# mynameisfiber/baton

Measured on NVIDIA H100. Metric: federated local samples/sec (whole box), ResNet-18 FedAvg, synthetic non-IID 32x32 shards, higher is better.
Workload: dtype bf16

## Files before the change

### baton_b200/csrc/bindings.cpp

```cpp
#include <ATen/cuda/CUDAContext.h>
#include <c10/cuda/CUDAGuard.h>
#include <torch/extension.h>

#include <optional>
#include <vector>

#include "launch.h"

namespace {

inline cudaStream_t cur_stream() { return at::cuda::getCurrentCUDAStream().stream(); }
inline void check(int rc, const char* what) {
  TORCH_CHECK(rc == 0, "baton_b200::", what, " failed with code ", rc,
              rc > 0 ? std::string(" (") + cudaGetErrorString(static_cast<cudaError_t>(rc)) + ")" : std::string());
}
inline const void* cptr(const at::Tensor& t) { return t.data_ptr(); }
inline void* ptr(at::Tensor& t) { return t.data_ptr(); }
template <class T>
inline T* opt_ptr(const std::optional<at::Tensor>& t) {
  return (t.has_value() && t->defined()) ? reinterpret_cast<T*>(t->data_ptr()) : nullptr;
}
#define CHECK_CUDA(x) TORCH_CHECK((x).is_cuda(), #x " must be a CUDA tensor")

inline const float* prox_anchor(const std::optional<at::Tensor>& anchor, int64_t numel, const at::Tensor& hyper) {
// ... 230 lines not shown
  TORCH_CHECK(rows > 0 && out.numel() % rows == 0, "conv_halo: out must hold [N*Ho*Wo, Nout] elements");
  const int64_t nout = out.numel() / rows;
  TORCH_CHECK(w.numel() == (dgrad ? c * 9 * nout : nout * 9 * c), "conv_halo: w must be [Cout, 9*Cin]");
  TORCH_CHECK(dgrad ? !col_stats.has_value()
                    : (!col_stats.has_value() || (col_stats->scalar_type() == at::kFloat && col_stats->numel() >= 2 * nout)),
              "conv_halo: col_stats is a [2 Cout] fp32 buffer of the forward");
  const c10::cuda::CUDAGuard guard(src.device());
  const int rc = b200_conv_halo(cptr(src), cptr(w), ptr(out), static_cast<int>(src.size(0)), static_cast<int>(src.size(1)),
                                static_cast<int>(src.size(2)), static_cast<int>(c), static_cast<int>(nout),
                                static_cast<int>(stride), dgrad ? 1 : 0, static_cast<int>(mc), opt_ptr<float>(col_stats),
                                cur_stream());
  if (rc == -2) return false;
  check(rc, "conv_halo");
  return true;
}
bool conv_igemm_dgrad_s2(const at::Tensor& dy, const at::Tensor& w, at::Tensor dx, int64_t kh, int64_t kw,
                         const std::vector<int64_t>& ntaps, const std::vector<int64_t>& taps, int64_t force_bn) {
  CHECK_CUDA(dy); CHECK_CUDA(w); CHECK_CUDA(dx);
  TORCH_CHECK(dy.scalar_type() == at::kBFloat16 && w.scalar_type() == at::kBFloat16 && dx.scalar_type() == at::kBFloat16 &&
              dy.dim() == 4 && dx.dim() == 4 && dy.is_contiguous() && w.is_contiguous() && dx.is_contiguous());
  TORCH_CHECK(ntaps.size() == 4 && taps.size() == 16, "conv_igemm_dgrad_s2: 4 classes x 4 taps");
  int nt[4], tw[16];
  for (int i = 0; i < 4; ++i) nt[i] = static_cast<int>(ntaps[i]);
  for (int i = 0; i < 16; ++i) tw[i] = static_cast<int>(taps[i]);
  const c10::cuda::CUDAGuard guard(dy.device());
  const int rc = b200_conv_igemm_dgrad_s2(cptr(dy), cptr(w), ptr(dx), static_cast<int>(dx.size(0)),
                                          static_cast<int>(dx.size(1)), static_cast<int>(dx.size(2)),
                                          static_cast<int>(dx.size(3)), static_cast<int>(dy.size(3)), static_cast<int>(kh),
                                          static_cast<int>(kw), static_cast<int>(dy.size(1)), static_cast<int>(dy.size(2)),
                                          nt, tw, static_cast<int>(force_bn), cur_stream());
  if (rc == -2) return false;
  check(rc, "conv_igemm_dgrad_s2");
  return true;
}
bool conv_igemm_wgrad(const at::Tensor& dy, const at::Tensor& x, at::Tensor dw, int64_t cout, int64_t kh, int64_t kw,
                      int64_t stride, int64_t pad, int64_t ho, int64_t wo, int64_t split_k, int64_t force_bn,
                      const std::optional<at::Tensor>& sgd_theta, const std::optional<at::Tensor>& sgd_theta_bf16,
                      const std::optional<at::Tensor>& sgd_mom, const std::optional<at::Tensor>& sgd_hyper,
                      bool sgd_nesterov, const std::optional<at::Tensor>& sgd_anchor,
                      const std::optional<at::Tensor>& sgd_corr, const std::optional<at::Tensor>& sgd_v) {
  CHECK_CUDA(dy); CHECK_CUDA(x); CHECK_CUDA(dw);
  TORCH_CHECK(x.scalar_type() == at::kBFloat16 && dy.scalar_type() == at::kBFloat16 && dw.scalar_type() == at::kFloat &&
              x.dim() == 4 && x.is_contiguous() && dy.is_contiguous());
  const c10::cuda::CUDAGuard guard(x.device());
  const std::optional<B200SgdEpilogue> sgd =
      sgd_epilogue(sgd_theta, sgd_theta_bf16, sgd_mom, sgd_hyper, sgd_nesterov, sgd_anchor, sgd_corr, sgd_v);
  const int rc = b200_conv_igemm_wgrad(cptr(dy), cptr(x), dw.data_ptr<float>(), static_cast<int>(x.size(0)),
                                       static_cast<int>(x.size(1)), static_cast<int>(x.size(2)), static_cast<int>(x.size(3)),
                                       static_cast<int>(cout), static_cast<int>(kh), static_cast<int>(kw),
                                       static_cast<int>(stride), static_cast<int>(pad), static_cast<int>(ho),
                                       static_cast<int>(wo), static_cast<int>(split_k), static_cast<int>(force_bn),
                                       sgd ? &*sgd : nullptr, cur_stream());
  if (rc == -2 || rc == B200_SGD_EPILOGUE_DECLINED) return false;
  check(rc, "conv_igemm_wgrad");
  return true;
}

void gemm_fp8(const at::Tensor& a, const at::Tensor& b, at::Tensor d, const std::optional<at::Tensor>& bias,
              const std::optional<at::Tensor>& sfa, const std::optional<at::Tensor>& sfb, int64_t M, int64_t N, int64_t K,
              int64_t lda, int64_t ldb, int64_t ldd, int64_t act, int64_t split_k, bool accumulate, double alpha) {
  CHECK_CUDA(a); CHECK_CUDA(b); CHECK_CUDA(d);
  TORCH_CHECK(a.element_size() == 1 && b.element_size() == 1, "gemm_fp8 operands must be 1-byte (e4m3)");
  const c10::cuda::CUDAGuard guard(a.device());
  check(b200_gemm_fp8(cptr(a), cptr(b), ptr(d), opt_ptr<const float>(bias), opt_ptr<const void>(sfa),
                      opt_ptr<const void>(sfb), M, N, K, lda, ldb, ldd, d.scalar_type() == at::kFloat, act, split_k,
                      accumulate, static_cast<float>(alpha), cur_stream()),
// ... 865 lines not shown
                                       loss_acc.data_ptr<float>(), opt_ptr<float>(logits_out), static_cast<int>(x.size(0)),
                                       static_cast<int>(x.size(1)), static_cast<int>(w.size(0)), cur_stream());
  if (rc == -2) return false;
  check(rc, "linear_xent_eval");
  return true;
}
void mse(const at::Tensor& pred, const at::Tensor& target, const std::optional<at::Tensor>& dpred, at::Tensor loss_acc,
         double grad_scale) {
  CHECK_CUDA(pred);
  TORCH_CHECK(target.scalar_type() == at::kFloat && target.numel() == pred.numel());
  const c10::cuda::CUDAGuard guard(pred.device());
  const int in32 = pred.scalar_type() == at::kFloat;
  const int out32 = dpred.has_value() && dpred->defined() && dpred->scalar_type() == at::kFloat;
  check(b200_mse(pred.data_ptr(), in32, target.data_ptr<float>(), opt_ptr<void>(dpred), out32,
                 loss_acc.data_ptr<float>(), pred.numel(), static_cast<float>(grad_scale), cur_stream()),
        "mse");
}

}

PYBIND11_MODULE(TORCH_EXTENSION_NAME, m) {
  m.doc() = "baton_b200 sm_90a kernels";
  m.attr("MAX_RANKS") = B200_MAX_RANKS;
  m.def("gemm", &gemm);
  m.def("trace_set", &trace_set);
  m.def("attention_fwd", &attention_fwd);
  m.def("attention_bwd", &attention_bwd);
  m.def("bn_bwd_cluster", &bn_bwd_cluster);
  m.def("im2col_tma_probe", &im2col_tma_probe);
  m.def("conv_igemm_fwd", &conv_igemm_fwd);
  m.def("conv_igemm_wgrad", &conv_igemm_wgrad);
  m.def("conv_igemm_dgrad", &conv_igemm_dgrad);
  m.def("conv_igemm_dgrad_s2", &conv_igemm_dgrad_s2);
  m.def("conv_halo", &conv_halo);
  m.def("gemm_batched", &gemm_batched);
  m.def("gemm_fp8", &gemm_fp8);
  m.def("quant_mx_rows", &quant_mx_rows);
  m.def("quant_mx_cols", &quant_mx_cols);
  m.def("fused_sgd", &fused_sgd);
  m.def("fused_sgd_segments", &fused_sgd_segments);
  m.def("weighted_sum", &weighted_sum);
  m.def("fold_client", &fold_client);
  m.def("scaffold_corr", &scaffold_corr);
  m.def("scaffold_dc", &scaffold_dc);
  m.def("cast", &cast);
  m.def("gather_rows", &gather_rows);
  m.def("gather_augment", &gather_augment);
  m.def("gather_mix", &gather_mix);
  m.def("colsum", &colsum);
  m.def("add_bf16", &add_bf16);
  m.def("relu_bwd", &relu_bwd);
  m.def("gelu", &gelu);
  m.def("gelu_bwd", &gelu_bwd);
  m.def("pad_rows", &pad_rows);
  m.def("embedding_bwd", &embedding_bwd);
  m.def("fedavg_allreduce", &fedavg_allreduce);
  m.def("fedavg_allreduce_robust", &fedavg_allreduce_robust);
  m.def("fedavg_allreduce_krum", &fedavg_allreduce_krum);
  m.attr("KRUM_MAX_CTAS") = B200_KRUM_MAX_CTAS;
  m.attr("KRUM_PAIRS") = B200_KRUM_PAIRS;
  m.attr("KRUM_REPORT") = B200_KRUM_REPORT;
  m.def("fedavg_allreduce_topk", &fedavg_allreduce_topk);
  m.def("fedavg_allreduce_local", &fedavg_allreduce_local);
  m.def("topk_pack", &topk_pack);
  m.def("topk_fold", &topk_fold);
  m.def("nonzero_pack", &nonzero_pack);
// ... 31 lines not shown
```

### baton_b200/csrc/gemm_wgmma.cu

```cuda
#define B200_TU_TAG 1
#include "ptx.cuh"
#include "epilogue.cuh"
#include "launch.h"
#include "pdl.cuh"
#include "sgd.cuh"

namespace b200 {

constexpr int BM = 128;
constexpr int BK = 64;
constexpr int WG_K = 16;
constexpr int GEMM_THREADS = 384;
constexpr int CONSUMER_WARPS = 8;
constexpr int CONSUMER_THREADS = 32 * CONSUMER_WARPS;
constexpr int MAX_STAGES = 8;
constexpr int S2_MAX_TAPS = 4;

struct GemmParams {
  int M, N, K;
  void* D;
  long long ldd;
  const float* bias;
  int out_fp32;
  int act;
  float* col_stats;
  int a_mn, b_mn;
  int k_tiles_per_split;
  int atomic_out;
  int cluster_k;
  int stages;
  const uint32_t* tile_flags;
  uint32_t flag_epoch;
  long long flag_elem_off;
  int flag_tile_elems;
  long long flag_bias_off;
  long long ldb;
  float alpha;
  int batched, batch_inner;
  int batch_count;
  long long d_outer, d_inner;
  int conv_ho, conv_wo;
  int conv_stride, conv_pad;
  int conv_kw;
  int conv_cin;
  int conv_taps;
  int conv_ncol;
  const uint32_t* flag_epoch_ptr;
  const float* sgd_hyper = nullptr;
  float* sgd_theta = nullptr;
  __nv_bfloat16* sgd_wb = nullptr;
  float* sgd_mom = nullptr;
  int sgd_nesterov = 0;
  int conv_h = 0, conv_w = 0;
  int s2_ntaps[4] = {0, 0, 0, 0};
  int s2_tap[4][S2_MAX_TAPS] = {};
  const float* bn_scale = nullptr;
  const float* bn_shift = nullptr;
  const __nv_bfloat16* residual = nullptr;
  long long ldr = 0;
  const float* sgd_anchor = nullptr;
  const float* sgd_corr = nullptr;
  float* sgd_v = nullptr;
};

__device__ __forceinline__ void wait_arrival_flags(const uint32_t* flags, long long e0, long long e1, int granule,
                                                   uint32_t need) {
  for (long long t = e0 / granule; t <= e1 / granule; ++t) {
    unsigned long long spins = 0;
    while (static_cast<int32_t>(ld_acquire_sys(flags + t) - need) < 0) {
      if (++spins > (1ull << 26)) break;
    }
  }
}

template <int BN>
struct SmemLayout {
  static constexpr int A_BYTES = BM * BK * 2;
  static constexpr int B_BYTES = BN * BK * 2;
  static constexpr int STAGE_BYTES = A_BYTES + B_BYTES;
  static constexpr int PART_PITCH = BN + 4;
  static constexpr int PART_BYTES = BM * PART_PITCH * 4;
};

__device__ __forceinline__ float apply_act(float v, int act) {
  if (act == 1) return fmaxf(v, 0.f);
  if (act == 2) {
    const float k0 = 0.7978845608028654f, k1 = 0.044715f;
    float t = tanhf(k0 * (v + k1 * v * v * v));
    return 0.5f * v * (1.f + t);
  }
  return v;
}

__device__ __forceinline__ float4 ld_dsmem_f4(uint32_t local_smem_addr, uint32_t cta_rank) {
  uint32_t remote;
// ... 256 lines not shown
__device__ __forceinline__ int s2_ntaps(const GemmParams& p, int cls) {
  int n = 0;
#pragma unroll
  for (int c = 0; c < 4; ++c) n = c == cls ? p.s2_ntaps[c] : n;
  return n;
}
__device__ __forceinline__ int s2_tap(const GemmParams& p, int cls, int slot) {
  int w = 0;
#pragma unroll
  for (int c = 0; c < 4; ++c)
#pragma unroll
    for (int t = 0; t < S2_MAX_TAPS; ++t) w = (c == cls && t == slot) ? p.s2_tap[c][t] : w;
  return w;
}
__device__ __forceinline__ int s2_dx_row(const GemmParams& p, int cls, int m) {
  if (m >= p.M) return -1;
  const int hw = p.conv_ho * p.conv_wo;
  const int n = m / hw, r = m - n * hw;
  const int i = r / p.conv_wo, j = r - i * p.conv_wo;
  const int h = 2 * i + (cls >> 1), w = 2 * j + (cls & 1);
  return (h < p.conv_h && w < p.conv_w) ? (n * p.conv_h + h) * p.conv_w + w : -1;
}
template <int BN>
__device__ __forceinline__ void s2_load_ktile(const CUtensorMap* tmA, const CUtensorMap* tmB, const GemmParams& p,
                                              uint8_t* sa, uint8_t* sb, uint64_t* bar, int cls, int kt, int m0, int n0) {
  const int cblocks = p.conv_cin >> 6;
  const int slot = kt / cblocks, cb = kt - slot * cblocks;
  const int tw = s2_tap(p, cls, slot);
  const int q0 = m0 % p.conv_wo, t0 = m0 / p.conv_wo;
  tma_load_im2col_4d(sa, tmA, bar, cb * 64, q0, t0 % p.conv_ho, t0 / p.conv_ho, (tw >> 24) & 0xff, (tw >> 16) & 0xff);
  const int wcol = (tw & 0xffff) * p.conv_ncol + n0;
#pragma unroll
  for (int j = 0; j < BN / 64; ++j) tma_load_2d(sb + j * 8192, tmB, bar, wcol + j * 64, cb * 64);
}

template <int BN, int STAGES, int CONV = 0, bool SGD = false, bool AFFINE = false, bool PROX = false, bool SCAF = false,
          bool ADAM = false>
__global__ void __launch_bounds__(GEMM_THREADS, 1)
gemm_bf16_fixed_kernel(const __grid_constant__ CUtensorMap tmA, const __grid_constant__ CUtensorMap tmB,
                         const GemmParams p) {
  using L = SmemLayout<BN>;
  static_assert(STAGES * L::STAGE_BYTES >= L::PART_BYTES, "the drained ring must hold the fp32 accumulator tile");
  extern __shared__ __align__(1024) uint8_t smem_raw[];
  uint8_t* smem = reinterpret_cast<uint8_t*>((reinterpret_cast<uintptr_t>(smem_raw) + 1023) & ~uintptr_t(1023));
  uint64_t* full_bar = reinterpret_cast<uint64_t*>(smem + STAGES * L::STAGE_BYTES);
  uint64_t* empty_bar = full_bar + STAGES;
  float* cstat = reinterpret_cast<float*>(empty_bar + STAGES);

  griddep_launch_dependents();
  const int warp = threadIdx.x >> 5;
  int m0 = blockIdx.y * BM;
  const int cls = CONV == 4 ? s2_class(p, m0) : 0;
  const int n0 = blockIdx.x * BN;
  const int k_tiles_total = CONV == 4 ? s2_ntaps(p, cls) * (p.conv_cin >> 6) : (p.K + BK - 1) / BK;
  const int bz_outer = p.batched ? static_cast<int>(blockIdx.z) / p.batch_inner : 0;
  const int bz_inner = p.batched ? static_cast<int>(blockIdx.z) % p.batch_inner : 0;
  const int kt_begin = p.batched ? 0 : blockIdx.z * p.k_tiles_per_split;
  int kt_end = kt_begin + p.k_tiles_per_split;
  if (kt_end > k_tiles_total) kt_end = k_tiles_total;
  const int num_kt = kt_end - kt_begin;

  if (warp == 0 && elect_one()) {
    tma_prefetch_desc(&tmA);
    tma_prefetch_desc(&tmB);
    for (int s = 0; s < STAGES; ++s) {
      mbar_init(&full_bar[s], 1);
// ... 18 lines not shown
        fence_proxy_async_all();
      }
      TRACE_POINT();
      for (int i = 0; i < num_kt; ++i) {
        const int s = i % STAGES;
        const uint32_t ph = (i / STAGES) & 1;
        mbar_wait(&empty_bar[s], ph ^ 1);
        uint8_t* sa = smem + s * L::STAGE_BYTES;
        uint8_t* sb = sa + L::A_BYTES;
        const int k0 = (kt_begin + i) * BK;
        if constexpr (CONV == 2) {
          const int live = (p.N - n0 + 63) / 64 < BN / 64 ? (p.N - n0 + 63) / 64 : BN / 64;
          mbar_expect_tx(&full_bar[s], L::A_BYTES + live * 8192);
        } else {
          mbar_expect_tx(&full_bar[s], L::STAGE_BYTES);
        }
        if (p.batched) {
          if (!p.a_mn) {
            tma_load_4d(sa, &tmA, &full_bar[s], k0, m0, bz_inner, bz_outer);
          } else {
#pragma unroll
            for (int j = 0; j < BM / 64; ++j)
              tma_load_4d(sa + j * 8192, &tmA, &full_bar[s], m0 + j * 64, k0, bz_inner, bz_outer);
          }
          if (!p.b_mn) {
            tma_load_4d(sb, &tmB, &full_bar[s], k0, n0, bz_inner, bz_outer);
          } else {
#pragma unroll
            for (int j = 0; j < BN / 64; ++j)
              tma_load_4d(sb + j * 8192, &tmB, &full_bar[s], n0 + j * 64, k0, bz_inner, bz_outer);
          }
        } else if constexpr (CONV == 4) {
          s2_load_ktile<BN>(&tmA, &tmB, p, sa, sb, &full_bar[s], cls, kt_begin + i, m0, n0);
        } else {
        if constexpr (CONV == 1 || CONV == 3) {
          const int kt = kt_begin + i;
          const int cblocks = p.conv_cin >> 6;
          const int tap = kt / cblocks, cb = kt - tap * cblocks;
          const int fr = tap / p.conv_kw, fs = tap - fr * p.conv_kw;
          const int q0 = m0 % p.conv_wo, t0 = m0 / p.conv_wo;
          tma_load_im2col_4d(sa, &tmA, &full_bar[s], cb * 64, q0 * p.conv_stride - p.conv_pad,
                             (t0 % p.conv_ho) * p.conv_stride - p.conv_pad, t0 / p.conv_ho, fs, fr);
        } else if (!p.a_mn) {
          tma_load_2d(sa, &tmA, &full_bar[s], k0, m0);
        } else {
#pragma unroll
          for (int j = 0; j < BM / 64; ++j)
            tma_load_2d(sa + j * 8192, &tmA, &full_bar[s], m0 + j * 64, k0);
        }
        if constexpr (CONV == 2) {
          const int q0 = k0 % p.conv_wo, t0 = k0 / p.conv_wo;
          const int w0 = q0 * p.conv_stride - p.conv_pad, h0 = (t0 % p.conv_ho) * p.conv_stride - p.conv_pad;
          const int img = t0 / p.conv_ho;
#pragma unroll
          for (int j = 0; j < BN / 64; ++j) {
            const int col = n0 + j * 64;
            if (col < p.N) {
              const int tap = col / p.conv_cin, c = col - tap * p.conv_cin;
              const int fr = tap / p.conv_kw, fs = tap - fr * p.conv_kw;
              tma_load_im2col_4d(sb + j * 8192, &tmB, &full_bar[s], c, w0, h0, img, fs, fr);
            }
          }
        } else if constexpr (CONV == 3) {
          const int kt = kt_begin + i;
          const int cblocks = p.conv_cin >> 6;
          const int tap = kt / cblocks, cb = kt - tap * cblocks;
// ... 78 lines not shown
          _Pragma("unroll") for (int j = 0; j < 32; ++j) if (col0 + j < p.N) atomicAdd(d + j, v[j]);
        }
      } else if (p.out_fp32) {
        float* d = reinterpret_cast<float*>(drow) + col0;
        if (full && vec_ok) {
#pragma unroll
          for (int j = 0; j < 32; j += 4)
            *reinterpret_cast<float4*>(d + j) = make_float4(v[j], v[j + 1], v[j + 2], v[j + 3]);
        } else {
          _Pragma("unroll") for (int j = 0; j < 32; ++j) if (col0 + j < p.N) d[j] = v[j];
        }
      } else {
        __nv_bfloat16* d = reinterpret_cast<__nv_bfloat16*>(drow) + col0;
        if (full && vec_ok) {
#pragma unroll
          for (int j = 0; j < 32; j += 8) {
            uint4 o;
            o.x = pack_bf16x2(v[j], v[j + 1]);
            o.y = pack_bf16x2(v[j + 2], v[j + 3]);
            o.z = pack_bf16x2(v[j + 4], v[j + 5]);
            o.w = pack_bf16x2(v[j + 6], v[j + 7]);
            *reinterpret_cast<uint4*>(d + j) = o;
          }
        } else {
          _Pragma("unroll") for (int j = 0; j < 32; ++j) if (col0 + j < p.N) d[j] = __float2bfloat16_rn(v[j]);
        }
      }
    }
    if (threadIdx.x == 128) TRACE_POINT();
    if (want_stats) {
      named_bar_sync(1, CONSUMER_THREADS);
      for (int i = threadIdx.x - 128; i < 2 * BN; i += CONSUMER_THREADS) {
        const int col = i < BN ? i : i - BN;
        if (n0 + col < p.N)
          atomicAdd(p.col_stats + (i < BN ? 0 : p.N) + n0 + col,
                    cstat[i] + cstat[2 * BN + i] + cstat[4 * BN + i] + cstat[6 * BN + i]);
      }
    }
  }
}


constexpr int EPI_PITCH = 144;
constexpr int EPI_WARP_BYTES = 32 * EPI_PITCH;

template <int BN>
__device__ __forceinline__ void epilogue_tile(const GemmParams& p, const float* acc_tile, int q, int half, int m0,
                                              int n0, uint8_t* stage, bool vec_ok, size_t d_off = 0) {
  using L = SmemLayout<BN>;
  const int lane = static_cast<int>(lane_id());
  const int row = m0 + q * 32 + lane;
  const float* arow = acc_tile + (q * 32 + lane) * L::PART_PITCH;
  const int elt = p.out_fp32 ? 4 : 2;
  const bool fast = vec_ok && !p.atomic_out && (p.N % 8 == 0);
  if (!fast) {
#pragma unroll 1
    for (int c = half * 32; c < BN; c += 64) {
      uint32_t r[32];
      acc_ld_row32(arow + c, r);
      const int col0 = n0 + c;
      if (col0 >= p.N) continue;
      float v[32];
#pragma unroll
      for (int j = 0; j < 32; ++j) v[j] = __uint_as_float(r[j]);
      if (p.col_stats != nullptr) accumulate_col_stats(p, col0, v);
      if (row >= p.M) continue;
      store_row_chunk<32>(p, row, col0, v, vec_ok, d_off);
// ... 180 lines not shown
  }
  __syncthreads();
  griddep_wait();

  if (warp == 0) {
    if (elect_one()) {
      if (p.tile_flags != nullptr) {
        const int rows_here = (p.N - n0) < BN ? (p.N - n0) : BN;
        const uint32_t need = p.flag_epoch_ptr != nullptr ? *reinterpret_cast<const volatile uint32_t*>(p.flag_epoch_ptr)
                                                          : p.flag_epoch;
        wait_arrival_flags(p.tile_flags, p.flag_elem_off + static_cast<long long>(n0) * p.ldb,
                           p.flag_elem_off + static_cast<long long>(n0 + rows_here) * p.ldb - 1, p.flag_tile_elems, need);
        if (p.flag_bias_off >= 0)
          wait_arrival_flags(p.tile_flags, p.flag_bias_off + n0, p.flag_bias_off + n0 + rows_here - 1,
                             p.flag_tile_elems, need);
        fence_proxy_async_all();
      }
      int s = 0;
      uint32_t ph = 0;
      for (int i = 0; i < num_kt; ++i) {
        mbar_wait(&empty_bar[s], ph ^ 1);
        uint8_t* sa = smem + s * L::STAGE_BYTES;
        uint8_t* sb = sa + L::A_BYTES;
        const int k0 = (kt_begin + i) * BK;
        mbar_expect_tx(&full_bar[s], L::STAGE_BYTES);
        if constexpr (CONV == 1 || CONV == 3) {
          const int kt = kt_begin + i;
          const int cblocks = p.conv_cin >> 6;
          const int tap = kt / cblocks, cb = kt - tap * cblocks;
          const int fr = tap / p.conv_kw, fs = tap - fr * p.conv_kw;
          const int q0 = m0 % p.conv_wo, t0 = m0 / p.conv_wo;
          tma_load_im2col_4d(sa, &tmA, &full_bar[s], cb * 64, q0 * p.conv_stride - p.conv_pad,
                             (t0 % p.conv_ho) * p.conv_stride - p.conv_pad, t0 / p.conv_ho, fs, fr);
        } else if (!p.a_mn) {
          tma_load_2d(sa, &tmA, &full_bar[s], k0, m0);
        } else {
#pragma unroll
          for (int j = 0; j < BM / 64; ++j)
            tma_load_2d(sa + j * 8192, &tmA, &full_bar[s], m0 + j * 64, k0);
        }
        if constexpr (CONV == 3) {
          const int kt = kt_begin + i;
          const int cblocks = p.conv_cin >> 6;
          const int tap = kt / cblocks, cb = kt - tap * cblocks;
          const int wcol = (p.conv_taps - 1 - tap) * p.conv_ncol + n0;
#pragma unroll
          for (int j = 0; j < BN / 64; ++j) tma_load_2d(sb + j * 8192, &tmB, &full_bar[s], wcol + j * 64, cb * 64);
        } else if (!p.b_mn) {
          tma_load_2d(sb, &tmB, &full_bar[s], k0, n0);
        } else {
#pragma unroll
          for (int j = 0; j < BN / 64; ++j) tma_load_2d(sb + j * 8192, &tmB, &full_bar[s], n0 + j * 64, k0);
        }
        if (++s == STAGES) { s = 0; ph ^= 1; }
      }
    }
  } else if (warp >= 4) {
    const int ew = warp - 4;
    float acc[BN / 2];
    int s = 0;
    uint32_t ph = 0;
    consume_ktiles<BN>(acc, smem, STAGES, full_bar, empty_bar, s, ph, num_kt, p.a_mn, p.b_mn, ew >> 2);
    named_bar_sync(1, CONSUMER_THREADS);
    float* part = reinterpret_cast<float*>(smem);
    wg_store_acc<BN>(acc, part, L::PART_PITCH, 64 * (ew >> 2));
    if constexpr (!CLUSTER) {
      named_bar_sync(1, CONSUMER_THREADS);
      const int q = ew & 3;
      constexpr int NCHUNK = BN / 32;
      const int c_begin = (ew < 4 ? 0 : (NCHUNK + 1) / 2) * 32, c_end = (ew < 4 ? (NCHUNK + 1) / 2 : NCHUNK) * 32;
      const int lrow = q * 32 + static_cast<int>(lane_id());
      const int row = m0 + lrow;
      const size_t elt = p.out_fp32 ? 4 : 2;
      const bool vec_ok = ((reinterpret_cast<uintptr_t>(p.D) & 15) == 0) && ((p.ldd * elt) % 16 == 0);
#pragma unroll 1
      for (int c = c_begin; c < c_end; c += 32) {
        const int col0 = n0 + c;
        if (row >= p.M || col0 >= p.N) continue;
        uint32_t r[32];
        acc_ld_row32(part + lrow * L::PART_PITCH + c, r);
// ... 28 lines not shown
          v[4] += b.x; v[5] += b.y; v[6] += b.z; v[7] += b.w;
        }
        const int row = m0 + lrow, col0 = n0 + c;
        if (want_stats) {
#pragma unroll
          for (int j = 0; j < 8; ++j) {
            const float rnd = __bfloat162float(__float2bfloat16_rn(v[j]));
            cs[j] += rnd;
            cq[j] = fmaf(rnd, rnd, cq[j]);
          }
        }
        if (row < p.M && col0 < p.N) store_row_chunk<8, AFFINE>(p, row, col0, v, vec_ok);
      }
      if (want_stats) {
#pragma unroll
        for (int j = 0; j < 8; ++j) {
#pragma unroll
          for (int o = CG; o < 32; o <<= 1) {
            cs[j] += __shfl_xor_sync(0xffffffffu, cs[j], o);
            cq[j] += __shfl_xor_sync(0xffffffffu, cq[j], o);
          }
        }
        const int wq = t >> 5, ln = t & 31;
        if (ln < CG) {
#pragma unroll
          for (int j = 0; j < 8; ++j) {
            cstat[wq * 2 * BN + ln * 8 + j] = cs[j];
            cstat[wq * 2 * BN + BN + ln * 8 + j] = cq[j];
          }
        }
        named_bar_sync(2, 128);
        for (int i = t; i < 2 * BN; i += 128) {
          const int col = i < BN ? i : i - BN;
          if (n0 + col < p.N) {
            const float v = cstat[i] + cstat[2 * BN + i] + cstat[4 * BN + i] + cstat[6 * BN + i];
            atomicAdd(p.col_stats + (i < BN ? 0 : p.N) + n0 + col, v);
          }
        }
      }
    }
    cluster_sync_all();
  }
}


typedef CUresult (*EncodeTiledFn)(CUtensorMap*, CUtensorMapDataType, cuuint32_t, void*, const cuuint64_t*,
                                  const cuuint64_t*, const cuuint32_t*, const cuuint32_t*, CUtensorMapInterleave,
                                  CUtensorMapSwizzle, CUtensorMapL2promotion, CUtensorMapFloatOOBfill);

static EncodeTiledFn get_encode_fn() {
  static thread_local bool ctx_bound = false;
  if (!ctx_bound) {
    cudaFree(nullptr);
    ctx_bound = true;
  }
  static EncodeTiledFn fn = nullptr;
  if (fn == nullptr) {
    void* ptr = nullptr;
    cudaDriverEntryPointQueryResult qres;
    cudaError_t e = cudaGetDriverEntryPoint("cuTensorMapEncodeTiled", &ptr, cudaEnableDefault, &qres);
    if (e != cudaSuccess || qres != cudaDriverEntryPointSuccess || ptr == nullptr) return nullptr;
    fn = reinterpret_cast<EncodeTiledFn>(ptr);
  }
  return fn;
}

static int make_map(CUtensorMap* map, const void* base, long long rows, long long cols, long long ld, int box_cols,
// ... 425 lines not shown
  int max_taps = 0;
  for (int c = 0; c < 4; ++c) {
    if (ntaps[c] < 0 || ntaps[c] > S2_MAX_TAPS) return -2;
    for (int t = 0; t < ntaps[c]; ++t) {
      const int tw = taps[c * S2_MAX_TAPS + t];
      if (tw < 0 || (tw & 0xffff) >= KH * KW) return -2;
      p.s2_tap[c][t] = tw;
    }
    p.s2_ntaps[c] = ntaps[c];
    max_taps = ntaps[c] > max_taps ? ntaps[c] : max_taps;
  }
  if (max_taps == 0) return -2;
  const int bn = clamp_bn(force_bn > 0 ? force_bn : (Cin > 64 ? 128 : 64));
  CUtensorMap ta, tb;
  int rc = b200_encode_map_im2col_bf16(&ta, dy, N, Ho, Wo, Cout, 1, 1, 1, 0, 64, BM);
  if (rc) return rc;
  rc = make_map(&tb, w, Cout, static_cast<long long>(KH) * KW * Cin, static_cast<long long>(KH) * KW * Cin, 64, BK);
  if (rc) return rc;
  const int k_tiles = max_taps * (Cout / 64);
  p.M = static_cast<int>(M); p.N = Cin; p.K = k_tiles * BK; p.D = dx; p.ldd = Cin; p.bias = nullptr; p.out_fp32 = 0;
  p.act = 0; p.a_mn = 0; p.b_mn = 1; p.k_tiles_per_split = k_tiles; p.cluster_k = 1; p.atomic_out = 0;
  p.col_stats = nullptr;
  p.tile_flags = nullptr; p.flag_epoch = 0; p.alpha = 1.0f; p.flag_elem_off = 0; p.flag_tile_elems = 0;
  p.ldb = static_cast<long long>(KH) * KW * Cin;
  p.flag_bias_off = -1; p.flag_epoch_ptr = nullptr;
  p.batched = 0; p.batch_inner = 1; p.batch_count = 1; p.d_outer = 0; p.d_inner = 0;
  p.conv_ho = Ho; p.conv_wo = Wo; p.conv_stride = 2; p.conv_pad = 0; p.conv_kw = KW; p.conv_cin = Cout;
  p.conv_taps = KH * KW; p.conv_ncol = Cin; p.conv_h = H; p.conv_w = W;
  dim3 grid((Cin + bn - 1) / bn, static_cast<unsigned>(4 * tiles_m), 1);
  if (bn == 128) return launch_fixed<128, 6, 4>(ta, tb, p, grid, stream);
  return launch_fixed<64, 8, 4>(ta, tb, p, grid, stream);
}

extern "C" int b200_conv_igemm_wgrad(const void* dy, const void* x, float* dw, int N, int H, int W, int Cin, int Cout,
                                     int KH, int KW, int stride, int pad, int Ho, int Wo, int split_k, int force_bn,
                                     const B200SgdEpilogue* sgd, cudaStream_t stream) {
  using namespace b200;
  const long long Mp = static_cast<long long>(N) * Ho * Wo;
  const int Kc = KH * KW * Cin;
  if (Mp <= 0 || Cout <= 0) return 0;
  if (Cin % 64 != 0 || Cout % 8 != 0 || Mp > (1ll << 30) || (reinterpret_cast<uintptr_t>(x) & 15) ||
      (reinterpret_cast<uintptr_t>(dy) & 15) || (reinterpret_cast<uintptr_t>(dw) & 15))
    return -2;
  const int bn = clamp_bn(force_bn > 0 ? force_bn : (Kc > 64 ? 128 : 64));
  CUtensorMap ta, tb;
  int rc = make_map(&ta, dy, Mp, Cout, Cout, 64, BK);
  if (rc) return rc;
  rc = b200_encode_map_im2col_bf16(&tb, x, N, H, W, Cin, KH, KW, stride, pad, 64, 64);
  if (rc) return rc;
  const int k_tiles = static_cast<int>((Mp + BK - 1) / BK);
  if (split_k < 1) split_k = 1;
  if (split_k > k_tiles) split_k = k_tiles;
  const int per = (k_tiles + split_k - 1) / split_k;
  split_k = (k_tiles + per - 1) / per;
  if (sgd != nullptr && split_k != 1) return B200_SGD_EPILOGUE_DECLINED;
  GemmParams p;
  if (sgd != nullptr) set_sgd_epilogue(p, *sgd);
  p.M = Cout; p.N = Kc; p.K = static_cast<int>(Mp); p.D = dw; p.ldd = Kc; p.bias = nullptr; p.out_fp32 = 1; p.act = 0;
  p.a_mn = 1; p.b_mn = 1; p.k_tiles_per_split = per; p.cluster_k = 1; p.atomic_out = 1;
  p.col_stats = nullptr;
  p.tile_flags = nullptr; p.flag_epoch = 0; p.alpha = 1.0f; p.flag_elem_off = 0; p.flag_tile_elems = 0; p.ldb = Kc;
  p.flag_bias_off = -1; p.flag_epoch_ptr = nullptr;
  p.batched = 0; p.batch_inner = 1; p.batch_count = 1; p.d_outer = 0; p.d_inner = 0;
  p.stages = 4;
  p.conv_ho = Ho; p.conv_wo = Wo; p.conv_stride = stride; p.conv_pad = pad; p.conv_kw = KW; p.conv_cin = Cin;
  p.conv_taps = KH * KW; p.conv_ncol = Cin;
// ... 11 lines not shown
```

### baton_b200/csrc/launch.h

```cpp
#pragma once
#include <cuda_runtime.h>
#include <stdint.h>

#define B200_MAX_RANKS 16

extern "C" {

struct B200SgdEpilogue {
  float* theta;
  void* theta_bf16;
  float* mom;
  const float* hyper;
  int nesterov;
  const float* anchor;
  const float* corr;
  float* v;
};
#define B200_SGD_EPILOGUE_DECLINED (-6)

struct B200AffineEpilogue {
  const float* scale;
  const float* shift;
  const void* residual;
  long long ldr;
  int relu;
};
#define B200_AFFINE_EPILOGUE_DECLINED (-7)

int b200_gemm_bf16(const void* a, const void* b, void* d, const float* bias, int M, int N, int K, long long lda,
                   long long ldb, long long ldd, int a_mn, int b_mn, int out_fp32, int act, int split_k, int accumulate,
                   float alpha, const uint32_t* tile_flags, uint32_t flag_epoch, long long flag_elem_off, int flag_tile_elems,
                   long long flag_bias_off, int force_bn, float* col_stats, const uint32_t* flag_epoch_ptr,
                   const B200SgdEpilogue* sgd, const B200AffineEpilogue* affine, cudaStream_t stream);
int b200_gemm_bf16_batched(const void* a, const void* b, void* d, int M, int N, int K, long long lda, long long ldb,
                           long long ldd, int a_mn, int b_mn, int out_fp32, int act, float alpha, int n_outer,
                           int n_inner, long long a_outer, long long a_inner, long long b_outer, long long b_inner,
                           long long d_outer, long long d_inner, int accumulate, cudaStream_t stream);
int b200_attention_fwd(const void* qkv, void* out, void* probs, int B, int S, int H, int dh, float scale,
                       cudaStream_t stream);
int b200_attention_bwd(const void* qkv, const void* dout, const void* probs, void* dqkv, int B, int S, int H, int dh,
                       float scale, cudaStream_t stream);
int b200_conv_igemm_fwd(const void* x, const void* w, void* y, int N, int H, int W, int Cin, int Cout, int KH, int KW,
                        int stride, int pad, int Ho, int Wo, int cluster_k, int force_bn, float* col_stats,
                        const B200AffineEpilogue* affine, cudaStream_t stream);
int b200_conv_igemm_dgrad(const void* dy, const void* w, void* dx, int N, int H, int W, int Cin, int Cout, int KH, int KW,
                          int pad, int Ho, int Wo, int cluster_k, int force_bn, cudaStream_t stream);
int b200_conv_igemm_dgrad_s2(const void* dy, const void* w, void* dx, int N, int H, int W, int Cin, int Cout, int KH,
                             int KW, int Ho, int Wo, const int* ntaps, const int* taps, int force_bn, cudaStream_t stream);
int b200_conv_igemm_wgrad(const void* dy, const void* x, float* dw, int N, int H, int W, int Cin, int Cout, int KH, int KW,
                          int stride, int pad, int Ho, int Wo, int split_k, int force_bn, const B200SgdEpilogue* sgd,
                          cudaStream_t stream);
int b200_conv_halo(const void* src, const void* w, void* out, int N, int H, int W, int C, int Nout, int stride,
                   int dgrad, int mc, float* col_stats, cudaStream_t stream);
int b200_im2col_tma_probe(const void* x, void* col, int N, int H, int W, int C, int KH, int KW, int stride, int pad,
                          int Ho, int Wo, cudaStream_t stream);
int b200_gemm_fp8(const void* a, const void* b, void* d, const float* bias, const void* sfa, const void* sfb, int M, int N,
                  int K, long long lda, long long ldb, long long ldd, int out_fp32, int act, int split_k, int accumulate,
                  float alpha, cudaStream_t stream);
int b200_quant_mx_rows(const void* x, void* q, void* sf, long long R, int C, long long ld_in, int Cp, cudaStream_t stream);
int b200_quant_mx_cols(const void* x, void* q, void* sf, long long R, int C, long long ld_in, long long Rp,
                       cudaStream_t stream);
int b200_gemm_simt(const void* a, const void* b, void* d, const float* bias, int M, int N, int K, long long lda,
                   long long ldb, long long ldd, int a_mn, int b_mn, int out_fp32, int act, int accumulate,
                   float alpha, cudaStream_t stream);

int b200_fused_sgd(float* w, float* g, float* mom, void* w_bf16, long long n, const float* hyper, int zero_grad,
                   int nesterov, const unsigned long long* wire_slot, const float* pack_global,
                   const float* pack_scale, long long n_pack, int wire_fp32, const float* prox_anchor,
                   const float* corr, float* adam_v, cudaStream_t stream);
int b200_fused_sgd_segments(float* w, float* g, float* mom, void* w_bf16, const long long* segments, int n_seg,
                            const float* hyper, int nesterov, const float* prox_anchor, const float* corr,
                            float* adam_v, cudaStream_t stream);
int b200_scaffold_corr(float* corr, const float* c, const float* ci, long long n, cudaStream_t stream);
int b200_scaffold_dc(float* up, float* ci, const float* c, const float* global_w, const float* theta, long long n,
                     float inv_k_eta, int first, cudaStream_t stream);
int b200_fold_client(float* acc, float* theta, const float* global_w, void* w_bf16, float* mom, long long n_mom, long long n,
                     float nk, int mode, int reset, cudaStream_t stream);
int b200_weighted_sum(void* dst, const void* const* srcs, const float* weights, int n_src, long long n, int dtype,
                      cudaStream_t stream);
int b200_cast_f32_bf16(const float* src, void* dst, long long n, cudaStream_t stream);
int b200_cast_bf16_f32(const void* src, float* dst, long long n, cudaStream_t stream);
// ... 182 lines not shown
```

### baton_b200/ops/functional.py

```python
from __future__ import annotations

import collections
import functools
from typing import List, Optional, Sequence, Tuple

import torch

from ._ext import load

BF16 = torch.bfloat16
NUM_SMS = 132


def _pitch(t: torch.Tensor) -> int:
    assert t.dim() == 2 and (t.stride(1) == 1 or t.shape[1] == 1), "GEMM operand must have unit inner stride"
    return t.stride(0) if t.shape[0] > 1 else max(t.stride(0), t.shape[1])


def _tma_ok(t: torch.Tensor) -> bool:
    return t.dtype == BF16 and _pitch(t) % 8 == 0 and t.data_ptr() % 16 == 0


def pick_bn(M: int, N: int) -> int:
    m_tiles = (M + 127) // 128
# ... 377 lines not shown
    gk = {}
    if gate is not None and form != "centre":
        gk = dict(flags=gate["flags"], flag_epoch_word=gate["epoch_word"], flag_elem_off=gate["elem_off"],
                  flag_tile_elems=gate["tile_elems"], force_bn=pick_bn(a.shape[0], w2d.shape[0]))
    return gemm(a, plan.weight(w2d), col_stats=col_stats, affine=affine, **gk), a


HALO_BM = 64
_HALO_MAX_SMEM = 227 * 1024
_HALO_FORMS = ((1, 64), (1, 128), (2, 64))


def halo_smem_bytes(h: int, w: int, c: int = 64, stride: int = 1) -> int:
    ho, wo = conv_out_size(h, 3, stride, 1), conv_out_size(w, 3, stride, 1)
    box = (HALO_BM // (ho * wo)) * (stride * (ho - 1) + 3) * (stride * (wo - 1) + 3) * 128
    k_tiles = 9 * (c // 64)
    return c // 64 * round_up(box, 1024) + k_tiles * 8192 + round_up(1 + k_tiles, 16) * 8 + 4 * 64 * 4 + 1024


def halo_eligible(kh: int, kw: int, stride: int, pad: int, c: int, h: int, w: int,
                  affine: Optional[dict] = None, dgrad: bool = False) -> bool:
    if kh != 3 or kw != 3 or pad != 1 or (stride, c) not in _HALO_FORMS or (dgrad and stride != 1):
        return False
    hw = conv_out_size(h, 3, stride, 1) * conv_out_size(w, 3, stride, 1)
    return (hw <= HALO_BM and HALO_BM % hw == 0 and affine is None and
            halo_smem_bytes(h, w, c, stride) <= _HALO_MAX_SMEM)


def halo_cluster(m_rows: int) -> int:
    tiles = (m_rows + HALO_BM - 1) // HALO_BM
    return 4 if tiles % 4 == 0 else 2 if tiles % 2 == 0 else 1


def _conv_path(path: Optional[str], eligible: bool) -> str:
    if path is None:
        return "halo" if eligible else "im2col"
    if path not in ("halo", "im2col"):
        raise ValueError("path must be None, 'halo' or 'im2col', not {!r}".format(path))
    if path == "halo" and not eligible:
        raise ValueError("the halo kernel does not take this convolution (see halo_eligible)")
    return path


def conv_igemm_fwd(x: torch.Tensor, w2d: torch.Tensor, kh: int, kw: int, stride: int, pad: int,
                   col_stats: Optional[torch.Tensor] = None, affine: Optional[dict] = None,
                   cluster_k: Optional[int] = None, force_bn: int = 0,
                   out: Optional[torch.Tensor] = None, path: Optional[str] = None,
                   mc: Optional[int] = None) -> Optional[torch.Tensor]:
    n, h, w, c = x.shape
    cout = w2d.shape[0]
    if c % 64 or w2d.shape[1] != kh * kw * c or not x.is_contiguous() or not w2d.is_contiguous():
        return None
    ho, wo = conv_out_size(h, kh, stride, pad), conv_out_size(w, kw, stride, pad)
    M, K = n * ho * wo, kh * kw * c
    halo = halo_eligible(kh, kw, stride, pad, c, h, w, affine) and cout % 8 == 0
    if _conv_path(path, halo) == "halo":
        y = out if out is not None else torch.empty((M, cout), dtype=BF16, device=x.device)
        if not load().conv_halo(x, w2d, y, stride, False, mc or halo_cluster(M), col_stats):
            raise RuntimeError("conv_halo declined a convolution halo_eligible admits")
        return y
    bn = force_bn or pick_bn(M, cout)
    if cluster_k is None:
        cluster_k = pick_cluster_k(M, cout, K, bn)
    y = out if out is not None else torch.empty((M, cout), dtype=BF16, device=x.device)
    af = affine or {}
    ok = load().conv_igemm_fwd(x, w2d, y, kh, kw, stride, pad, ho, wo, cluster_k, bn, col_stats, af.get("scale"),
                               af.get("shift"), af.get("residual"), bool(af.get("relu", False)))
    return y if ok else None


S2_MAX_TAPS = 4


def conv_s2_dgrad_taps(kh: int, kw: int, pad: int, ho: int, wo: int) -> Optional[List[List[Tuple[int, int, int]]]]:
    classes = []
    for a in (0, 1):
        for b in (0, 1):
            taps = []
            for r in range(kh):
                if (a + pad - r) % 2:
                    continue
                dp = (a + pad - r) // 2
                for s in range(kw):
                    if (b + pad - s) % 2:
                        continue
                    dq = (b + pad - s) // 2
                    if dp < 0 or dq < 0:
                        return None
                    if dp < ho and dq < wo:
                        taps.append((r * kw + s, dp, dq))
            if len(taps) > S2_MAX_TAPS:
                return None
            classes.append(taps)
    return classes


def conv_igemm_dgrad(dy: torch.Tensor, w2d: torch.Tensor, in_shape, kh: int, kw: int, pad: int, stride: int = 1,
                     out: Optional[torch.Tensor] = None, path: Optional[str] = None,
                     mc: Optional[int] = None, cluster_k: Optional[int] = None) -> Optional[torch.Tensor]:
    n, h, w, c = in_shape
    cout = dy.shape[-1]
    if c % 64 or cout % 64 or w2d.shape[1] != kh * kw * c or not dy.is_contiguous() or not w2d.is_contiguous():
        return None
    if _conv_path(path, halo_eligible(kh, kw, stride, pad, cout, h, w, dgrad=True)) == "halo":
        dx = out if out is not None else torch.empty((n, h, w, c), dtype=BF16, device=dy.device)
        if not load().conv_halo(dy, w2d, dx, 1, True, mc or halo_cluster(n * h * w), None):
            raise RuntimeError("conv_halo declined a convolution halo_eligible admits")
        return dx
    if stride == 1:
        M, K = n * h * w, kh * kw * cout
        bn = pick_bn(M, c)
        dx = out if out is not None else torch.empty((n, h, w, c), dtype=BF16, device=dy.device)
        if cluster_k is None:
            cluster_k = pick_cluster_k(M, c, K, bn)
        ok = load().conv_igemm_dgrad(dy, w2d, dx, kh, kw, pad, cluster_k, bn)
        return dx if ok else None
    if stride != 2:
        return None
    ho, wo = dy.shape[1], dy.shape[2]
    classes = conv_s2_dgrad_taps(kh, kw, pad, ho, wo)
    if classes is None:
        return None
    bn = pick_bn(4 * n * ho * wo, c)
    words = [[t | dp << 16 | dq << 24 for t, dp, dq in taps] + [0] * (S2_MAX_TAPS - len(taps)) for taps in classes]
    dx = out if out is not None else torch.empty((n, h, w, c), dtype=BF16, device=dy.device)
    ok = load().conv_igemm_dgrad_s2(dy, w2d, dx, kh, kw, [len(t) for t in classes], [x for ws in words for x in ws], bn)
    return dx if ok else None


def conv_igemm_wgrad_(dy2d: torch.Tensor, x: torch.Tensor, dw2d: torch.Tensor, kh: int, kw: int, stride: int,
                      pad: int, sgd: Optional[dict] = None) -> bool:
    n, h, w, c = x.shape
    cout = dy2d.shape[1]
    if c % 64 or not x.is_contiguous() or not dy2d.is_contiguous() or not dw2d.is_contiguous():
        return False
    ho, wo = conv_out_size(h, kh, stride, pad), conv_out_size(w, kw, stride, pad)
    M, K = n * ho * wo, kh * kw * c
    bn = pick_bn(cout, K)
    split_k = pick_split_k(cout, K, M, bn)
    if sgd is not None and split_k != 1:
# ... 174 lines not shown
```

Measured before the change: 225,800.

## Add tap-gather GEMM path for 3x3 convs on tiny spatial maps

Adds a new conv kernel variant (CONV 5/6) for 3x3 pad-1 convolutions on maps of at most 2x2 pixels. Instead of im2col over nine taps, mostly padding zeros, it loads only the valid (pixel, tap) pairs, and output pixels become column groups of one GEMM. This cuts K from 9*Cin to at most 4*Cin for ResNet-18's last-stage 2x2 and 1x1 layers, for both forward and stride-1 dgrad. The cost is a new loader, a separate column-stats indexing path and host-side table building on every call. Correctness depends on the entry encoding and the grouping, both of which are intricate.

```diff
diff --git a/baton_b200/csrc/bindings.cpp b/baton_b200/csrc/bindings.cpp
--- a/baton_b200/csrc/bindings.cpp
+++ b/baton_b200/csrc/bindings.cpp
@@ -286,6 +286,39 @@
   if (rc == -2) return false;
   check(rc, "conv_igemm_dgrad_s2");
   return true;
+}
+static void conv_tap(const at::Tensor& a, const at::Tensor& w, at::Tensor d, int64_t cin, int64_t cout, bool dgrad,
+                     int64_t ngroups, int64_t nent, const std::vector<int64_t>& entries, int64_t cluster_k,
+                     int64_t force_bn, const std::optional<at::Tensor>& col_stats, const char* name) {
+  CHECK_CUDA(a); CHECK_CUDA(w); CHECK_CUDA(d);
+  TORCH_CHECK(a.scalar_type() == at::kBFloat16 && w.scalar_type() == at::kBFloat16 && d.scalar_type() == at::kBFloat16 &&
+              a.dim() == 4 && d.dim() == 4 && a.is_contiguous() && w.is_contiguous() && d.is_contiguous(), name,
+              ": bf16 contiguous NHWC tensors");
+  TORCH_CHECK(w.dim() == 2 && w.size(0) == cout && w.size(1) == 9 * cin, name, ": w must be [Cout, 9 Cin]");
+  TORCH_CHECK(a.size(3) == (dgrad ? cout : cin) && d.size(0) == a.size(0) &&
+              d.size(1) * d.size(2) == ngroups && d.size(3) == (dgrad ? cin : cout), name, ": operand shapes");
+  TORCH_CHECK(ngroups >= 1 && ngroups <= 4 && entries.size() == static_cast<size_t>(4 * ngroups), name,
+              ": 1 to 4 groups of 4 entry words");
+  TORCH_CHECK(!col_stats.has_value() || (col_stats->scalar_type() == at::kFloat && col_stats->numel() >= 2 * cout),
+              name, ": col_stats is a [2 Cout] fp32 buffer");
+  int ent[16];
+  for (size_t i = 0; i < entries.size(); ++i) ent[i] = static_cast<int>(entries[i]);
+  const c10::cuda::CUDAGuard guard(a.device());
+  const int rc = b200_conv_tap_gemm(cptr(a), cptr(w), ptr(d), static_cast<int>(a.size(0)), static_cast<int>(cin),
+                                    static_cast<int>(cout), 9, dgrad ? 1 : 0, static_cast<int>(a.size(1) * a.size(2)),
+                                    static_cast<int>(ngroups), static_cast<int>(nent), ent, static_cast<int>(cluster_k),
+                                    static_cast<int>(force_bn), opt_ptr<float>(col_stats), cur_stream());
+  check(rc, name);
+}
+void conv_tap_fwd(const at::Tensor& x, const at::Tensor& w, at::Tensor y, int64_t nent, const std::vector<int64_t>& entries,
+                  int64_t cluster_k, int64_t force_bn, const std::optional<at::Tensor>& col_stats) {
+  conv_tap(x, w, y, x.size(3), w.size(0), false, y.size(1) * y.size(2), nent, entries, cluster_k, force_bn, col_stats,
+           "conv_tap_fwd");
+}
+void conv_tap_dgrad(const at::Tensor& dy, const at::Tensor& w, at::Tensor dx, int64_t nent,
+                    const std::vector<int64_t>& entries, int64_t cluster_k, int64_t force_bn) {
+  conv_tap(dy, w, dx, dx.size(3), w.size(0), true, dx.size(1) * dx.size(2), nent, entries, cluster_k, force_bn,
+           std::nullopt, "conv_tap_dgrad");
 }
 bool conv_igemm_wgrad(const at::Tensor& dy, const at::Tensor& x, at::Tensor dw, int64_t cout, int64_t kh, int64_t kw,
                       int64_t stride, int64_t pad, int64_t ho, int64_t wo, int64_t split_k, int64_t force_bn,
@@ -1217,6 +1250,8 @@
   m.def("conv_igemm_wgrad", &conv_igemm_wgrad);
   m.def("conv_igemm_dgrad", &conv_igemm_dgrad);
   m.def("conv_igemm_dgrad_s2", &conv_igemm_dgrad_s2);
+  m.def("conv_tap_fwd", &conv_tap_fwd);
+  m.def("conv_tap_dgrad", &conv_tap_dgrad);
   m.def("conv_halo", &conv_halo);
   m.def("gemm_batched", &gemm_batched);
   m.def("gemm_fp8", &gemm_fp8);
diff --git a/baton_b200/csrc/gemm_wgmma.cu b/baton_b200/csrc/gemm_wgmma.cu
--- a/baton_b200/csrc/gemm_wgmma.cu
+++ b/baton_b200/csrc/gemm_wgmma.cu
@@ -15,6 +15,8 @@
 constexpr int CONSUMER_THREADS = 32 * CONSUMER_WARPS;
 constexpr int MAX_STAGES = 8;
 constexpr int S2_MAX_TAPS = 4;
+constexpr int TAP_MAX_GROUPS = 4;
+constexpr int TAP_MAX_ENTRIES = 4;
 
 struct GemmParams {
   int M, N, K;
@@ -61,6 +63,9 @@
   const float* sgd_anchor = nullptr;
   const float* sgd_corr = nullptr;
   float* sgd_v = nullptr;
+  int tap_group = 0;
+  int tap_nent = 0;
+  int tap_ent[4][4] = {};
 };
 
 __device__ __forceinline__ void wait_arrival_flags(const uint32_t* flags, long long e0, long long e1, int granule,
@@ -383,6 +388,31 @@
   const int wcol = (tw & 0xffff) * p.conv_ncol + n0;
 #pragma unroll
   for (int j = 0; j < BN / 64; ++j) tma_load_2d(sb + j * 8192, tmB, bar, wcol + j * 64, cb * 64);
+}
+
+__device__ __forceinline__ int tap_entry(const GemmParams& p, int grp, int e) {
+  int w = 0;
+#pragma unroll
+  for (int g = 0; g < TAP_MAX_GROUPS; ++g)
+#pragma unroll
+    for (int t = 0; t < TAP_MAX_ENTRIES; ++t) w = (g == grp && t == e) ? p.tap_ent[g][t] : w;
+  return w;
+}
+template <int BN, int CONV>
+__device__ __forceinline__ void tap_load_ktile(const CUtensorMap* tmA, const CUtensorMap* tmB, const GemmParams& p,
+                                               uint8_t* sa, uint8_t* sb, uint64_t* bar, int kt, int m0, int n0) {
+  const int cblocks = p.conv_cin >> 6;
+  const int e = kt / cblocks, cb = kt - e * cblocks;
+  const int grp = n0 / p.tap_group, nn = n0 - grp * p.tap_group;
+  const int tw = tap_entry(p, grp, e);
+  tma_load_2d(sa, tmA, bar, (tw & 0xffff) * p.conv_cin + cb * 64, m0);
+  const int wcol = (tw >> 16) * p.conv_ncol;
+  if constexpr (CONV == 5) {
+    tma_load_2d(sb, tmB, bar, wcol + cb * 64, nn);
+  } else {
+#pragma unroll
+    for (int j = 0; j < BN / 64; ++j) tma_load_2d(sb + j * 8192, tmB, bar, wcol + nn + j * 64, cb * 64);
+  }
 }
 
 template <int BN, int STAGES, int CONV = 0, bool SGD = false, bool AFFINE = false, bool PROX = false, bool SCAF = false,
@@ -467,6 +497,8 @@
           }
         } else if constexpr (CONV == 4) {
           s2_load_ktile<BN>(&tmA, &tmB, p, sa, sb, &full_bar[s], cls, kt_begin + i, m0, n0);
+        } else if constexpr (CONV == 5 || CONV == 6) {
+          tap_load_ktile<BN, CONV>(&tmA, &tmB, p, sa, sb, &full_bar[s], kt_begin + i, m0, n0);
         } else {
         if constexpr (CONV == 1 || CONV == 3) {
           const int kt = kt_begin + i;
@@ -611,7 +643,10 @@
       named_bar_sync(1, CONSUMER_THREADS);
       for (int i = threadIdx.x - 128; i < 2 * BN; i += CONSUMER_THREADS) {
         const int col = i < BN ? i : i - BN;
-        if (n0 + col < p.N)
+        if constexpr (CONV == 5) {
+          atomicAdd(p.col_stats + (i < BN ? 0 : p.tap_group) + n0 % p.tap_group + col,
+                    cstat[i] + cstat[2 * BN + i] + cstat[4 * BN + i] + cstat[6 * BN + i]);
+        } else if (n0 + col < p.N)
           atomicAdd(p.col_stats + (i < BN ? 0 : p.N) + n0 + col,
                     cstat[i] + cstat[2 * BN + i] + cstat[4 * BN + i] + cstat[6 * BN + i]);
       }
@@ -858,6 +893,8 @@
           const int q0 = m0 % p.conv_wo, t0 = m0 / p.conv_wo;
           tma_load_im2col_4d(sa, &tmA, &full_bar[s], cb * 64, q0 * p.conv_stride - p.conv_pad,
                              (t0 % p.conv_ho) * p.conv_stride - p.conv_pad, t0 / p.conv_ho, fs, fr);
+        } else if constexpr (CONV == 5 || CONV == 6) {
+          tap_load_ktile<BN, CONV>(&tmA, &tmB, p, sa, sb, &full_bar[s], kt_begin + i, m0, n0);
         } else if (!p.a_mn) {
           tma_load_2d(sa, &tmA, &full_bar[s], k0, m0);
         } else {
@@ -872,6 +909,7 @@
           const int wcol = (p.conv_taps - 1 - tap) * p.conv_ncol + n0;
 #pragma unroll
           for (int j = 0; j < BN / 64; ++j) tma_load_2d(sb + j * 8192, &tmB, &full_bar[s], wcol + j * 64, cb * 64);
+        } else if constexpr (CONV == 5 || CONV == 6) {
         } else if (!p.b_mn) {
           tma_load_2d(sb, &tmB, &full_bar[s], k0, n0);
         } else {
@@ -966,7 +1004,10 @@
         named_bar_sync(2, 128);
         for (int i = t; i < 2 * BN; i += 128) {
           const int col = i < BN ? i : i - BN;
-          if (n0 + col < p.N) {
+          if constexpr (CONV == 5) {
+            const float v = cstat[i] + cstat[2 * BN + i] + cstat[4 * BN + i] + cstat[6 * BN + i];
+            atomicAdd(p.col_stats + (i < BN ? 0 : p.tap_group) + n0 % p.tap_group + col, v);
+          } else if (n0 + col < p.N) {
             const float v = cstat[i] + cstat[2 * BN + i] + cstat[4 * BN + i] + cstat[6 * BN + i];
             atomicAdd(p.col_stats + (i < BN ? 0 : p.N) + n0 + col, v);
           }
@@ -1458,6 +1499,58 @@
   return launch_fixed<64, 8, 4>(ta, tb, p, grid, stream);
 }
 
+extern "C" int b200_conv_tap_gemm(const void* a, const void* w, void* d, int N, int Cin, int Cout, int taps, int dgrad,
+                                  int apix, int ngroups, int nent, const int* entries, int cluster_k, int force_bn, float* col_stats,
+                                  cudaStream_t stream) {
+  using namespace b200;
+  if (N <= 0) return 0;
+  const int ablk = dgrad ? Cout : Cin, group = dgrad ? Cin : Cout;
+  if (Cin % 64 != 0 || Cout % 64 != 0 || apix < 1 || apix > TAP_MAX_GROUPS || ngroups < 1 ||
+      ngroups > TAP_MAX_GROUPS || nent < 1 ||
+      nent > TAP_MAX_ENTRIES || (dgrad && col_stats != nullptr) || (reinterpret_cast<uintptr_t>(a) & 15) ||
+      (reinterpret_cast<uintptr_t>(w) & 15) || (reinterpret_cast<uintptr_t>(d) & 15))
+    return -2;
+  GemmParams p;
+  for (int g = 0; g < ngroups; ++g)
+    for (int e = 0; e < nent; ++e) {
+      const int tw = entries[g * TAP_MAX_ENTRIES + e];
+      if (tw < 0 || (tw & 0xffff) >= apix || (tw >> 16) >= taps) return -2;
+      p.tap_ent[g][e] = tw;
+    }
+  const int K = nent * ablk;
+  const long long ka = static_cast<long long>(apix) * ablk;
+  const int Nn = ngroups * group;
+  int bn = clamp_bn(force_bn > 0 ? force_bn : (Nn > 64 ? 128 : 64));
+  if (group % bn) bn = 64;
+  CUtensorMap ta, tb;
+  int rc = make_map(&ta, a, N, ka, ka, BK, BM);
+  if (rc) return rc;
+  const long long wk = static_cast<long long>(taps) * Cin;
+  rc = dgrad ? make_map(&tb, w, Cout, wk, wk, 64, BK) : make_map(&tb, w, Cout, wk, wk, BK, bn);
+  if (rc) return rc;
+  const int k_tiles = K / BK;
+  if (cluster_k != 1 && cluster_k != 2 && cluster_k != 4 && cluster_k != 8) return -5;
+  while (cluster_k > 1 && (cluster_k - 1) * ((k_tiles + cluster_k - 1) / cluster_k) >= k_tiles) cluster_k >>= 1;
+  const int per = (k_tiles + cluster_k - 1) / cluster_k;
+  p.M = N; p.N = Nn; p.K = K; p.D = d; p.ldd = Nn; p.bias = nullptr; p.out_fp32 = 0; p.act = 0;
+  p.a_mn = 0; p.b_mn = dgrad; p.k_tiles_per_split = per; p.cluster_k = cluster_k; p.atomic_out = 0;
+  p.col_stats = col_stats;
+  p.tile_flags = nullptr; p.flag_epoch = 0; p.alpha = 1.0f; p.flag_elem_off = 0; p.flag_tile_elems = 0; p.ldb = wk;
+  p.flag_bias_off = -1; p.flag_epoch_ptr = nullptr;
+  p.batched = 0; p.batch_inner = 1; p.batch_count = 1; p.d_outer = 0; p.d_inner = 0;
+  const int max_stages = bn == 128 ? 6 : 8;
+  p.stages = per < max_stages ? (per < 2 ? 2 : per) : max_stages;
+  p.conv_cin = ablk; p.conv_ncol = Cin; p.conv_taps = taps;
+  p.tap_group = group; p.tap_nent = nent;
+  dim3 grid(Nn / bn, static_cast<unsigned>((N + BM - 1) / BM), cluster_k);
+  if (dgrad) {
+    if (cluster_k > 1) return bn == 128 ? launch_cfg<128, 6>(ta, tb, p, grid, stream) : launch_cfg<64, 6>(ta, tb, p, grid, stream);
+    return bn == 128 ? launch_fixed<128, 6, 6>(ta, tb, p, grid, stream) : launch_fixed<64, 8, 6>(ta, tb, p, grid, stream);
+  }
+  if (cluster_k > 1) return bn == 128 ? launch_cfg<128, 5>(ta, tb, p, grid, stream) : launch_cfg<64, 5>(ta, tb, p, grid, stream);
+  return bn == 128 ? launch_fixed<128, 6, 5>(ta, tb, p, grid, stream) : launch_fixed<64, 8, 5>(ta, tb, p, grid, stream);
+}
+
 extern "C" int b200_conv_igemm_wgrad(const void* dy, const void* x, float* dw, int N, int H, int W, int Cin, int Cout,
                                      int KH, int KW, int stride, int pad, int Ho, int Wo, int split_k, int force_bn,
                                      const B200SgdEpilogue* sgd, cudaStream_t stream) {
diff --git a/baton_b200/csrc/launch.h b/baton_b200/csrc/launch.h
--- a/baton_b200/csrc/launch.h
+++ b/baton_b200/csrc/launch.h
@@ -47,6 +47,9 @@
                           int pad, int Ho, int Wo, int cluster_k, int force_bn, cudaStream_t stream);
 int b200_conv_igemm_dgrad_s2(const void* dy, const void* w, void* dx, int N, int H, int W, int Cin, int Cout, int KH,
                              int KW, int Ho, int Wo, const int* ntaps, const int* taps, int force_bn, cudaStream_t stream);
+int b200_conv_tap_gemm(const void* a, const void* w, void* d, int N, int Cin, int Cout, int taps, int dgrad, int apix,
+                       int ngroups, int nent, const int* entries, int cluster_k, int force_bn, float* col_stats,
+                       cudaStream_t stream);
 int b200_conv_igemm_wgrad(const void* dy, const void* x, float* dw, int N, int H, int W, int Cin, int Cout, int KH, int KW,
                           int stride, int pad, int Ho, int Wo, int split_k, int force_bn, const B200SgdEpilogue* sgd,
                           cudaStream_t stream);
diff --git a/baton_b200/ops/functional.py b/baton_b200/ops/functional.py
--- a/baton_b200/ops/functional.py
+++ b/baton_b200/ops/functional.py
@@ -433,14 +433,58 @@
     return 4 if tiles % 4 == 0 else 2 if tiles % 2 == 0 else 1
 
 
-def _conv_path(path: Optional[str], eligible: bool) -> str:
+TAP_MAX_GROUPS = 4
+
+
+def conv_tap_table(kh: int, kw: int, stride: int, pad: int, h: int, w: int,
+                   dgrad: bool = False) -> List[List[Tuple[int, int]]]:
+    ho, wo = conv_out_size(h, kh, stride, pad), conv_out_size(w, kw, stride, pad)
+    fwd = [[] for _ in range(ho * wo)]
+    for pos in range(ho * wo):
+        oi, oj = divmod(pos, wo)
+        for pix in range(h * w):
+            r, q = pix // w - oi * stride + pad, pix % w - oj * stride + pad
+            if 0 <= r < kh and 0 <= q < kw:
+                fwd[pos].append((pix, r * kw + q))
+    if not dgrad:
+        return fwd
+    groups = [[] for _ in range(h * w)]
+    for pos, entries in enumerate(fwd):
+        for pix, tap in entries:
+            groups[pix].append((pos, tap))
+    return groups
+
+
+def tap_gemm_eligible(kh: int, kw: int, stride: int, pad: int, c: int, cout: int, h: int, w: int,
+                      affine: Optional[dict] = None, dgrad: bool = False) -> bool:
+    if kh != 3 or kw != 3 or pad != 1 or c % 64 or cout % 64 or affine is not None:
+        return False
+    if stride not in (1, 2) or (dgrad and stride != 1) or h > 2 or w > 2:
+        return False
+    return not halo_eligible(kh, kw, stride, pad, cout if dgrad else c, h, w, dgrad=dgrad)
+
+
+def _conv_path(path: Optional[str], eligible: bool, taps: bool = False) -> str:
     if path is None:
-        return "halo" if eligible else "im2col"
-    if path not in ("halo", "im2col"):
-        raise ValueError("path must be None, 'halo' or 'im2col', not {!r}".format(path))
+        return "halo" if eligible else "taps" if taps else "im2col"
+    if path not in ("halo", "taps", "im2col"):
+        raise ValueError("path must be None, 'halo', 'taps' or 'im2col', not {!r}".format(path))
     if path == "halo" and not eligible:
         raise ValueError("the halo kernel does not take this convolution (see halo_eligible)")
+    if path == "taps" and not taps:
+        raise ValueError("the tap GEMM does not take this convolution (see tap_gemm_eligible)")
     return path
+
+
+def _tap_args(n: int, group: int, groups, dense_k: int, cluster_k: Optional[int], force_bn: int):
+    N = len(groups) * group
+    bn = force_bn or pick_bn(n, N)
+    if group % bn:
+        bn = 64
+    if cluster_k is None:
+        cluster_k = pick_cluster_k(n, N, dense_k, bn)
+    words = [x for g in groups for x in [pix | tap << 16 for pix, tap in g] + [0] * (TAP_MAX_GROUPS - len(g))]
+    return words, len(groups[0]), cluster_k, bn
 
 
 def conv_igemm_fwd(x: torch.Tensor, w2d: torch.Tensor, kh: int, kw: int, stride: int, pad: int,
@@ -455,10 +499,17 @@
     ho, wo = conv_out_size(h, kh, stride, pad), conv_out_size(w, kw, stride, pad)
     M, K = n * ho * wo, kh * kw * c
     halo = halo_eligible(kh, kw, stride, pad, c, h, w, affine) and cout % 8 == 0
-    if _conv_path(path, halo) == "halo":
+    which = _conv_path(path, halo, tap_gemm_eligible(kh, kw, stride, pad, c, cout, h, w, affine))
+    if which == "halo":
         y = out if out is not None else torch.empty((M, cout), dtype=BF16, device=x.device)
         if not load().conv_halo(x, w2d, y, stride, False, mc or halo_cluster(M), col_stats):
             raise RuntimeError("conv_halo declined a convolution halo_eligible admits")
+        return y
+    if which == "taps":
+        y = out if out is not None else torch.empty((M, cout), dtype=BF16, device=x.device)
+        groups = conv_tap_table(kh, kw, stride, pad, h, w)
+        words, nent, ck, bn = _tap_args(n, cout, groups, K, cluster_k, force_bn)
+        load().conv_tap_fwd(x, w2d, y.view(n, ho, wo, cout), nent, words, ck, bn, col_stats)
         return y
     bn = force_bn or pick_bn(M, cout)
     if cluster_k is None:
@@ -503,10 +554,18 @@
     cout = dy.shape[-1]
     if c % 64 or cout % 64 or w2d.shape[1] != kh * kw * c or not dy.is_contiguous() or not w2d.is_contiguous():
         return None
-    if _conv_path(path, halo_eligible(kh, kw, stride, pad, cout, h, w, dgrad=True)) == "halo":
+    which = _conv_path(path, halo_eligible(kh, kw, stride, pad, cout, h, w, dgrad=True),
+                       tap_gemm_eligible(kh, kw, stride, pad, c, cout, h, w, dgrad=True))
+    if which == "halo":
         dx = out if out is not None else torch.empty((n, h, w, c), dtype=BF16, device=dy.device)
         if not load().conv_halo(dy, w2d, dx, 1, True, mc or halo_cluster(n * h * w), None):
             raise RuntimeError("conv_halo declined a convolution halo_eligible admits")
+        return dx
+    if which == "taps":
+        dx = out if out is not None else torch.empty((n, h, w, c), dtype=BF16, device=dy.device)
+        groups = conv_tap_table(kh, kw, stride, pad, h, w, dgrad=True)
+        words, nent, ck, bn = _tap_args(n, c, groups, kh * kw * cout, cluster_k, 0)
+        load().conv_tap_dgrad(dy, w2d, dx, nent, words, ck, bn)
         return dx
     if stride == 1:
         M, K = n * h * w, kh * kw * cout
```

Result: faster. 229,200, median of 6 (+1.5%).
